# Fro116/RecommenderSystem

Measured on AMD Instinct MI355X. Metric: interactions/sec, higher is better.
Workload: dtype bf16

## Files before the change

include/rsys_debug.h:

```cpp
#ifndef RSYS_DEBUG_H
#define RSYS_DEBUG_H
#include "rsys.h"

#ifdef __cplusplus
extern "C" {
#endif

int32_t rsys_debug_get(rsys_model* m, const char* key, void* out, int64_t bytes);

int32_t rsys_local_group_create(int32_t world, int32_t device, void** group);
int32_t rsys_local_group_destroy(void* group);
int32_t rsys_comm_init_local(void* group, int32_t rank, rsys_comm** out);
int32_t rsys_comm_debug_delay(rsys_comm* c, int32_t microseconds);

int32_t rsys_dev_alloc(void** p, size_t bytes);
int32_t rsys_dev_free(void* p);
int32_t rsys_dev_h2d(void* dst, const void* src, size_t bytes);
int32_t rsys_dev_d2h(void* dst, const void* src, size_t bytes);
int32_t rsys_dev_memset(void* dst, int value, size_t bytes);
int32_t rsys_op_gemm(int32_t dtype, const void* A, const void* B, void* C, int32_t M, int32_t N, int32_t K,
                     int64_t lda, int64_t ldb, int64_t ldc, int32_t a_km, int32_t b_km, int32_t a_f32, int32_t c_f32,
                     int32_t splitk);
int32_t rsys_op_gemm_rows(int32_t dtype, const void* A, const void* B, void* C, int32_t M, int32_t N, int32_t K,
                          int64_t lda, int64_t ldb, int64_t ldc, int32_t b_km, int32_t c_f32, const int32_t* rows_dev);
int32_t rsys_op_gemm_klimit(int32_t dtype, const void* A, const void* B, void* C, int32_t M, int32_t N, int32_t K,
                            int64_t lda, int64_t ldb, int64_t ldc, int32_t accumulate, const int32_t* k_dev);
int32_t rsys_op_gemm_epi(int32_t dtype, const void* A, const void* B, void* C, int32_t M, int32_t N, int32_t K, int64_t lda,
                         int64_t ldb, int64_t ldc, int32_t b_km, int32_t c_f32, int32_t epi, float alpha, int32_t accum,
                         const float* bias, const float* resid, int64_t ldr, void* C2, int64_t ldc2, const float* E,
                         const float* rope_cos, const float* rope_sin, const float* rope_cs, const int32_t* rope_pos, int32_t T,
                         int32_t hd, int32_t n_q, int32_t n_k, const int32_t* m_dev, char* tag, int32_t tag_bytes, int32_t* half);
int32_t rsys_debug_gemm_route(int32_t dtype, int32_t M, int32_t N, int32_t K, int64_t lda, int64_t ldb, int64_t ldc, int32_t a_km,
                              int32_t b_km, int32_t a_f32, int32_t c_f32, int32_t epi, int32_t splitk, int32_t flags, float alpha,
                              int32_t accum, int32_t set, int32_t m_expect, int32_t cus, char* tag, int32_t tag_bytes, int32_t* splits);
int32_t rsys_op_attention(int32_t dtype, int32_t B, int32_t T, int32_t H, int32_t KV, int32_t hd, const void* qkv,
                          const int32_t* uid, const int32_t* tm, void* O, float* lse, const void* dO, void* dqkv,
                          const float* rope_cos, const float* rope_sin);
int32_t rsys_op_attention_ex(int32_t dtype, int32_t B, int32_t T, int32_t H, int32_t KV, int32_t hd, const void* qkv,
                             const int32_t* uid, const int32_t* tm, void* O, float* lse, const void* dO, void* dqkv,
                             const float* rope_cos, const float* rope_sin, const int32_t* rope_pos, int32_t rope_rows,
                             const int32_t* q_active, float* amax_fwd, float* amax_bwd);
int32_t rsys_op_attention_selected(int32_t dtype, int32_t B, int32_t T, int32_t H, int32_t KV, int32_t hd, const void* qkv,
                                   const int32_t* uid, const int32_t* tm, int32_t n_sel, const int32_t* sel, void* O);
int32_t rsys_op_attention_cached(int32_t dtype, int32_t rows, int32_t T, int32_t H, int32_t KV, int32_t hd, const void* qkv, const void* cache,
                                 int32_t n_slots, const int32_t* slot, const int32_t* n_hist, const int32_t* n_cand, void* O);
// ... 103 lines not shown
```

recommendersystem_amd/_lib.py:

```python
import ctypes as C
import os

os.environ.setdefault("HSA_ENABLE_IPC_MODE_LEGACY", "0")

HERE = os.path.dirname(os.path.abspath(__file__))
LIB_PATH = os.path.join(HERE, "librsys_hip.so")


class RsysError(RuntimeError):
    pass


class rsys_config(C.Structure):
    _fields_ = [
        ("num_layers", C.c_int32), ("num_heads", C.c_int32), ("num_kv_heads", C.c_int32),
        ("embed_dim", C.c_int32), ("intermediate_dim", C.c_int32), ("max_sequence_length", C.c_int32),
        ("vocab_0", C.c_int32), ("vocab_1", C.c_int32),
        ("vocab_status", C.c_int32), ("vocab_gender", C.c_int32), ("vocab_source", C.c_int32),
        ("metadata_dim", C.c_int32),
        ("min_ts", C.c_double), ("max_ts", C.c_double),
        ("rating_mean", C.c_float), ("rating_std", C.c_float), ("mask_rate", C.c_float),
        ("mask_topk", C.c_int32), ("finetune", C.c_int32), ("finetune_metric", C.c_int32),
        ("dtype", C.c_int32), ("max_rows", C.c_int32), ("lora_dropout", C.c_float),
        ("table_shard_rank", C.c_int32), ("table_shard_world", C.c_int32), ("sampled_negatives", C.c_int32),
# ... 165 lines not shown
    ("rsys_grad_sync_schedule", C.c_int32, [_P, C.POINTER(C.c_int64), C.c_int32, C.POINTER(C.c_int32)]),
    ("rsys_comm_info", C.c_int32, [_P, C.POINTER(C.c_int32)]),
    ("rsys_allreduce_f64", C.c_int32, [_P, C.POINTER(C.c_double), C.c_int32]),
    ("rsys_self_test", C.c_int32, [_P]),
    ("rsys_param_checksum", C.c_int32, [_P, C.POINTER(C.c_double * 4)]),
    ("rsys_grad_buffer", C.c_int32, [_P, C.POINTER(_P), C.POINTER(C.c_int64)]),
    ("rsys_param_buffer", C.c_int32, [_P, C.POINTER(_P), C.POINTER(C.c_int64)]),
    ("rsys_refresh_shadow", C.c_int32, [_P]),
    ("rsys_dev_alloc", C.c_int32, [C.POINTER(_P), C.c_size_t]),
    ("rsys_dev_free", C.c_int32, [_P]),
    ("rsys_dev_h2d", C.c_int32, [_P, _P, C.c_size_t]),
    ("rsys_dev_d2h", C.c_int32, [_P, _P, C.c_size_t]),
    ("rsys_dev_memset", C.c_int32, [_P, C.c_int, C.c_size_t]),
    ("rsys_op_gemm", C.c_int32, [C.c_int32, _P, _P, _P, C.c_int32, C.c_int32, C.c_int32, C.c_int64, C.c_int64, C.c_int64,
                                 C.c_int32, C.c_int32, C.c_int32, C.c_int32, C.c_int32]),
    ("rsys_op_f8_quantize", C.c_int32, [_P, C.c_int64, C.c_int32, C.c_int32, C.c_int32, C.c_int32, C.c_int32, C.c_int32, _P, C.c_int64, _P, _P, _P,
                                          C.c_int32, C.c_int32, C.c_int32]),
    ("rsys_op_f8_weights", C.c_int32, [_P, C.c_int64, C.c_int32, C.c_int32, C.c_int32, C.c_int32, C.c_int32, _P, _P, _P, C.c_int64]),
    ("rsys_op_gemm_f8", C.c_int32, [_P, _P, _P, C.c_int32, C.c_int32, C.c_int32, C.c_int64, C.c_int64, C.c_int64, C.c_int32, C.c_int32, _P,
                                      C.c_int32, C.c_int32, C.c_int32, C.c_int32, C.c_int32]),
    ("rsys_op_gemm_rows", C.c_int32, [C.c_int32, _P, _P, _P, C.c_int32, C.c_int32, C.c_int32, C.c_int64, C.c_int64, C.c_int64,
                                      C.c_int32, C.c_int32, _P]),
    ("rsys_op_gemm_klimit", C.c_int32, [C.c_int32, _P, _P, _P, C.c_int32, C.c_int32, C.c_int32, C.c_int64, C.c_int64, C.c_int64, C.c_int32, _P]),
    ("rsys_op_gemm_epi", C.c_int32, [C.c_int32, _P, _P, _P, C.c_int32, C.c_int32, C.c_int32, C.c_int64, C.c_int64, C.c_int64, C.c_int32, C.c_int32,
                                     C.c_int32, C.c_float, C.c_int32, _P, _P, C.c_int64, _P, C.c_int64, _P, _P, _P, _P, _P,
                                     C.c_int32, C.c_int32, C.c_int32, C.c_int32, _P, C.c_char_p, C.c_int32, C.POINTER(C.c_int32)]),
    ("rsys_debug_gemm_route", C.c_int32, [C.c_int32] * 4 + [C.c_int64] * 3 + [C.c_int32] * 7 + [C.c_float] + [C.c_int32] * 4
                                          + [C.c_char_p, C.c_int32, C.POINTER(C.c_int32)]),
    ("rsys_op_attention", C.c_int32, [C.c_int32] + [C.c_int32] * 5 + [_P] * 9),
    ("rsys_op_attention_ex", C.c_int32, [C.c_int32] + [C.c_int32] * 5 + [_P] * 10 + [C.c_int32, _P, _P, _P]),
    ("rsys_op_query_weights", C.c_int32, [_P, C.c_int64, _P, _P, _P, C.c_int32, _P, C.c_int32, _P, _P, C.c_int32, C.c_int32,
                                          _P, _P, _P, _P, _P, _P, C.c_float, C.c_int32, _P,
                                          _P, _P, _P, C.c_int32, _P, _P, C.c_int32, _P, _P]),
    ("rsys_op_topk", C.c_int32, [_P, C.c_int64, C.c_int32, C.c_int32, C.c_int32, _P, _P, _P]),
    ("rsys_op_topk_window", C.c_int32, [_P, C.c_int64, C.c_int32, C.c_int32, _P, _P, _P, _P, _P, _P, _P]),
    ("rsys_op_lse", C.c_int32, [_P, C.c_int64, C.c_int32, C.c_int32, _P]),
    ("rsys_op_target_rank", C.c_int32, [_P, C.c_int64, C.c_int32, C.c_int32, _P, _P]),
    ("rsys_op_pair_ranks", C.c_int32, [_P, C.c_int64, C.c_int32, C.c_int32, _P, _P, _P, _P]),
    ("rsys_rank_gram_get", C.c_int32, [_P, C.c_int32, C.c_int32, _P, _P, _P, C.c_int64]),
    ("rsys_op_rerank", C.c_int32, [C.c_int32, C.c_int32, _P, _P, _P, _P, _P, _P]),
    ("rsys_op_embedding_scatter", C.c_int32, [_P, C.c_int64, _P, _P, C.c_int32, C.c_int32, C.c_int32, _P, C.c_int32]),
    ("rsys_op_rmsnorm_fwd", C.c_int32, [C.c_int32, _P, _P, _P, _P, C.c_int64, C.c_int32, _P, _P, _P]),
    ("rsys_op_rmsnorm_bwd", C.c_int32, [C.c_int32, C.c_int32] + [_P] * 11 + [C.c_int64, C.c_int32, _P, C.c_int32]),
    ("rsys_op_ce", C.c_int32, [C.c_int32, _P, C.c_int64, C.c_int32, C.c_int32] + [_P] * 6 + [C.c_float, _P, C.c_int32]),
    ("rsys_op_rating_tail", C.c_int32, [C.c_int32, _P, _P, C.c_int32, C.c_int32] + [_P] * 6 + [C.c_float, C.c_float, C.c_int32]
                                        + [_P] * 5 + [C.c_int32]),
# ... 77 lines not shown
```

recommendersystem_amd/csrc/capi.hip:

```cpp
#include <algorithm>
#include <dlfcn.h>
#include <math.h>
#include <stdlib.h>
#include <string.h>

#include <sstream>

#include "comm.hpp"
#include "encoder_handle.hpp"
#include "model_internal.hpp"

namespace rsys {
static thread_local std::string g_err;
void set_error(const std::string& msg) { g_err = msg; }
}

using namespace rsys;

struct rsys_model { Model* m; };
struct rsys_optimizer { Optimizer o; };

#define CHECK_HANDLE(h) do { if ((h) == nullptr) { set_error("null handle"); return RSYS_ERR_ARG; } } while (0)

namespace {
// ... 829 lines not shown
  return RSYS_OK;
}
int32_t rsys_param_buffer(rsys_model* h, void** p, int64_t* n) { CHECK_HANDLE(h); *p = h->m->P; *n = h->m->n_total; return RSYS_OK; }
int32_t rsys_refresh_shadow(rsys_model* h) { CHECK_HANDLE(h); return model_refresh_shadow(h->m); }

int32_t rsys_dev_alloc(void** p, size_t bytes) { HIP_CHECK(hipMalloc(p, bytes ? bytes : 16)); HIP_CHECK(hipMemset(*p, 0, bytes ? bytes : 16)); return RSYS_OK; }
int32_t rsys_dev_free(void* p) { HIP_CHECK(hipFree(p)); return RSYS_OK; }
int32_t rsys_dev_h2d(void* d, const void* s, size_t n) { HIP_CHECK(hipMemcpy(d, s, n, hipMemcpyHostToDevice)); return RSYS_OK; }
int32_t rsys_dev_d2h(void* d, const void* s, size_t n) { HIP_CHECK(hipDeviceSynchronize()); HIP_CHECK(hipMemcpy(d, s, n, hipMemcpyDeviceToHost)); return RSYS_OK; }
int32_t rsys_dev_memset(void* d, int v, size_t n) { HIP_CHECK(hipMemset(d, v, n)); return RSYS_OK; }

int32_t rsys_op_gemm(int32_t dtype, const void* A, const void* B, void* C, int32_t M, int32_t N, int32_t K, int64_t lda,
                     int64_t ldb, int64_t ldc, int32_t a_km, int32_t b_km, int32_t a_f32, int32_t c_f32, int32_t splitk) {
  switches_parse();
  GemmParams p{};
  p.A = A; p.B = B; p.C = C; p.M = M; p.N = N; p.K = K; p.lda = lda; p.ldb = ldb; p.ldc = ldc;
  p.c_f32 = c_f32; p.splitk = splitk < 1 ? 1 : splitk; p.alpha = 1.f;
  p.epi = p.splitk > 1 ? EPI_ATOMIC : EPI_STORE;
  if (sw().debug_epi >= 0) p.epi = sw().debug_epi;
  int rc = dtype == RSYS_DTYPE_BF16 ? launch_gemm<bf16>(p, a_f32 != 0, false, a_km != 0, b_km != 0, nullptr)
                                    : launch_gemm<float>(p, false, false, a_km != 0, b_km != 0, nullptr);
  if (rc) return rc;
  HIP_CHECK(hipDeviceSynchronize());
  return RSYS_OK;
}

int32_t rsys_op_gemm_rows(int32_t dtype, const void* A, const void* B, void* C, int32_t M, int32_t N, int32_t K, int64_t lda,
                          int64_t ldb, int64_t ldc, int32_t b_km, int32_t c_f32, const int32_t* rows_dev) {
  switches_parse();
  ARG_CHECK(rows_dev != nullptr, "rsys_op_gemm_rows: rows_dev is null");
  GemmParams p{};
  p.A = A; p.B = B; p.C = C; p.M = M; p.N = N; p.K = K; p.lda = lda; p.ldb = ldb; p.ldc = ldc;
  p.c_f32 = c_f32 != 0; p.splitk = 1; p.alpha = 1.f; p.epi = EPI_STORE; p.m_dev = rows_dev;
  if (c_f32 == 3) { p.epi = EPI_ATOMIC; p.splitk = 8; }
  int rc = dtype == RSYS_DTYPE_BF16 ? launch_gemm<bf16>(p, false, false, false, b_km != 0, nullptr)
                                    : launch_gemm<float>(p, false, false, false, b_km != 0, nullptr);
  if (rc) return rc;
  HIP_CHECK(hipDeviceSynchronize());
  return RSYS_OK;
}

int32_t rsys_op_gemm_klimit(int32_t dtype, const void* A, const void* B, void* C, int32_t M, int32_t N, int32_t K, int64_t lda,
                            int64_t ldb, int64_t ldc, int32_t accumulate, const int32_t* k_dev) {
  switches_parse();
  ARG_CHECK(k_dev != nullptr, "rsys_op_gemm_klimit: k_dev is null");
  GemmParams p{};
// ... 963 lines not shown
```

recommendersystem_amd/csrc/gemm.hpp:

```cpp
#pragma once
#include "common.hpp"

namespace rsys {

enum GemmEpi : int {
  EPI_STORE = 0,
  EPI_ACCUM = 1,
  EPI_ATOMIC = 2,
  EPI_BIAS = 3,
  EPI_RESIDUAL = 4,
  EPI_QKV_ROPE = 5,
  EPI_SWIGLU = 6,
  EPI_TABLE = 7,
  EPI_GELU = 8,
  EPI_SWIGLU_BWD = 9
};

enum GemmFlag : int {
  GEMM_NO_STORE_ALLOWANCE = 1 << 0,
  GEMM_ONE_WG_PER_TILE = 1 << 1,
  GEMM_START_STAGGER = 1 << 2,
  GEMM_BAND_SHIFT = 3,
  GEMM_BAND_MASK = 15 << GEMM_BAND_SHIFT,
  GEMM_SPLITK_256 = 1 << 7,
// ... 27 lines not shown
  int f8_seg_cols;
  int f8_alt;
  int f8_kb[3];
  float* f8_amax_out;
  int f8_rseg;
  int f8_rowmode;
};

template <typename CT>
int launch_gemm(const GemmParams& p, bool a_f32, bool b_f32, bool a_km, bool b_km, hipStream_t s);

enum GemmKernel : int { GK_NT, GK_NN, GK_TN, GK_8P, GK_8C, GK_4P, GK_8T, GK_4K, GK_8TS, GK_8S, GK_8M, GK_COUNT };
extern const char* const gemm_kernel_tags[GK_COUNT];
struct GemmRoute { GemmKernel kernel; int splitk; };
template <typename CT>
GemmRoute gemm_route(const GemmParams& p, bool a_f32, bool b_f32, bool a_km, bool b_km, int cus);

template <typename CT>
long long gemm_slab_need(const GemmParams& p, bool a_f32, bool b_f32, bool a_km, bool b_km);

struct GemmGroupPlan;
bool gemm8p_group_eligible(const GemmParams& p);
int gemm8p_group_plan_create(const GemmParams* probs, int n, GemmGroupPlan** out, bool ordered = false);
void gemm8p_group_plan_destroy(GemmGroupPlan* pl);
double gemm8p_group_flops(const GemmGroupPlan* pl);
bool gemm8p_group_on_4k(const GemmGroupPlan* pl);
int gemm8p_group_splitk(const GemmGroupPlan* pl);
int launch_gemm8p_group(const GemmGroupPlan* pl, hipStream_t s);

bool gemm8p_mix_eligible(const GemmParams& p);
int launch_gemm8p_mix(const GemmParams& p, hipStream_t s);
bool gemm8p_f8_eligible(const GemmParams& p);
int launch_gemm8p_f8(const GemmParams& p, hipStream_t s);
bool gemm8p_f8_splitk_eligible(const GemmParams& p);
int launch_gemm8p_f8_splitk(const GemmParams& p, hipStream_t s);

const char* gemm_kernel_name(const GemmParams& p, bool bf16_mode, bool a_f32, bool b_f32, bool a_km, bool b_km);
bool gemm8c_uses_half(const GemmParams& p, int cus);

}
```

recommendersystem_amd/csrc/gemm8p.hip:

```cpp
#include <algorithm>
#include <vector>

#include "gemm.hpp"
#include "gemm_epi.hpp"
#include "gemm_epi_reg.hpp"

namespace rsys {

#define GLB_AS __attribute__((address_space(1)))

namespace {

constexpr int T8_BM = 256, T8_BN = 256, T8_BK = 64;

typedef __attribute__((ext_vector_type(4))) int i32x4;
extern "C" __device__ void rsys_raw_buffer_load_lds(i32x4 rsrc, LDS_AS unsigned int* lds, int size, int voffset, int soffset,
                                                    int offset, int aux) __asm("llvm.amdgcn.raw.buffer.load.lds");

__device__ __forceinline__ i32x4 make_rsrc(const char* base) {
  const unsigned long long a = (unsigned long long)base;
  i32x4 r;
  r[0] = __builtin_amdgcn_readfirstlane((int)(unsigned int)a);
  r[1] = __builtin_amdgcn_readfirstlane((int)(unsigned int)((a >> 32) & 0xFFFFu));
  r[2] = -1;
// ... 495 lines not shown
  bool asm4k = false;
  double flops = 0.0;
  float* slab_all = nullptr; size_t slab_bytes = 0; int max_mn4 = 0;
};

__global__ void slab_reduce_group_kernel(const GemmParams* __restrict__ probs) {
  const GemmParams& p = probs[blockIdx.y];
  const long long n4 = (long long)p.M * p.N / 4, stride = (long long)p.M * p.N;
  float* C = (float*)p.C;
  for (long long i = (long long)blockIdx.x * blockDim.x + threadIdx.x; i < n4; i += (long long)gridDim.x * blockDim.x) {
    float4 acc = *(const float4*)(p.slab + 4 * i);
    for (int sp = 1; sp < p.splitk; ++sp) {
      const float4 v = *(const float4*)(p.slab + sp * stride + 4 * i);
      acc.x += v.x; acc.y += v.y; acc.z += v.z; acc.w += v.w;
    }
    const long long e = 4 * i, row = e / p.N; const int col = (int)(e % p.N);
    float4* c = (float4*)(C + row * p.ldc + col);
    float4 o = *c; o.x += acc.x; o.y += acc.y; o.z += acc.z; o.w += acc.w; *c = o;
  }
}

bool gemm8p_group_eligible(const GemmParams& p) { return (p.f8 ? gemm8p_f8_splitk_eligible(p) : gemm8p_tn_eligible(p)) && p.slab == nullptr; }

int gemm8p_group_plan_create(const GemmParams* probs, int n, GemmGroupPlan** out, bool ordered) {
  ARG_CHECK(n >= 1 && n <= 128, "grouped GEMM: 1..128 products");
  const int per_xcd = std::max(1, cu_count() / 8);
  std::vector<int> tiles(n), ktiles(n);
  int ktmax = 0;
  const bool f8 = probs[0].f8 != 0;
  for (int i = 0; i < n; ++i) {
    ARG_CHECK((probs[i].f8 != 0) == f8, "grouped GEMM: fp8 and bf16 products in one plan");
    ARG_CHECK(gemm8p_group_eligible(probs[i]), "grouped GEMM: product not eligible for the split-K LDS-DMA kernel");
    tiles[i] = ((probs[i].M + T8_BM - 1) / T8_BM) * ((probs[i].N + T8_BN - 1) / T8_BN);
    ARG_CHECK(tiles[i] < 65536, "grouped GEMM: too many tiles");
    ktiles[i] = f8 ? probs[i].K / 128 : (probs[i].K + T8_BK - 1) / T8_BK;
    ktmax = std::max(ktmax, ktiles[i]);
  }
  std::vector<int> order(n);
  for (int i = 0; i < n; ++i) order[i] = i;
  std::stable_sort(order.begin(), order.end(), [&](int a, int b) { return (long long)tiles[a] * ktiles[a] > (long long)tiles[b] * ktiles[b]; });
  std::vector<std::vector<int>> lists(8);
  long long load[8] = {0, 0, 0, 0, 0, 0, 0, 0};
  for (int i : order) {
    int best = 0;
    for (int x = 1; x < 8; ++x) if (load[x] < load[best]) best = x;
    lists[best].push_back(i); load[best] += (long long)tiles[i] * ktiles[i];
  }
  const int force = sw().debug_8g_splitk;
  int best_s = 1; double best_t = 1e300;
  for (int s = 1; s <= 16; ++s) {
    if (s > 1 && (ktmax + s - 1) / s < 8) break;
    double worst = 0.0;
    for (int x = 0; x < 8; ++x) {
      std::vector<double> slot(per_xcd, 0.0);
      for (int i : lists[x]) {
        const int per = (ktiles[i] + s - 1) / s;
        for (int sp = 0; sp < s; ++sp) {
          const int nt = std::min(ktiles[i], (sp + 1) * per) - sp * per;
          if (nt <= 0) continue;
          for (int t = 0; t < tiles[i]; ++t) { auto it = std::min_element(slot.begin(), slot.end()); *it += nt + 24.0; }
        }
      }
      worst = std::max(worst, *std::max_element(slot.begin(), slot.end()));
    }
    if (worst < best_t) { best_t = worst; best_s = s; }
  }
  if (force > 0) best_s = std::min(force, 255);
  std::vector<GemmParams> hp(probs, probs + n);
  std::vector<int> off(9, 0);
  std::vector<unsigned int> work;
  int longest = 0;
  double flops = 0.0;
  for (int i = 0; i < n; ++i) { hp[i].splitk = best_s; if (hp[i].alpha == 0.f) hp[i].alpha = 1.f; flops += 2.0 * hp[i].M * hp[i].N * (double)hp[i].K; }
  float* slab_all = nullptr; size_t slab_bytes = 0; int max_mn4 = 0;
  if (ordered) {
    ARG_CHECK(!f8, "grouped GEMM: the ordered form exists for the bf16 products only");
    long long total = 0;
    for (int i = 0; i < n; ++i) {
      ARG_CHECK(hp[i].N % 4 == 0 && hp[i].ldc % 4 == 0, "grouped GEMM: the ordered split-K sum needs N % 4 == 0");
      total += (long long)best_s * hp[i].M * hp[i].N;
      max_mn4 = std::max(max_mn4, (int)((long long)hp[i].M * hp[i].N / 4));
    }
    slab_bytes = (size_t)total * 4;
    if (hipMalloc((void**)&slab_all, slab_bytes) != hipSuccess) { set_error("grouped GEMM: hipMalloc of the split-K slabs failed"); return RSYS_ERR_HIP; }
    long long at = 0;
    for (int i = 0; i < n; ++i) { hp[i].slab = slab_all + at; hp[i].slab_floats = (long long)best_s * hp[i].M * hp[i].N; at += hp[i].slab_floats; }
  }
  for (int x = 0; x < 8; ++x) {
    off[x] = (int)work.size();
    for (int i : lists[x]) {
      const int per = (ktiles[i] + best_s - 1) / best_s;
      for (int sp = 0; sp < best_s; ++sp) {
        if (sp * per >= ktiles[i]) continue;
        for (int t = 0; t < tiles[i]; ++t) work.push_back(((unsigned int)i << 24) | ((unsigned int)sp << 16) | (unsigned int)t);
      }
    }
    longest = std::max(longest, (int)work.size() - off[x]);
  }
  off[8] = (int)work.size();
  GemmGroupPlan* pl = new GemmGroupPlan();
  const size_t b_probs = (sizeof(GemmParams) * n + 255) / 256 * 256, b_off = 256, b_work = (work.size() * 4 + 255) / 256 * 256;
  pl->slab_all = slab_all; pl->slab_bytes = slab_bytes; pl->max_mn4 = max_mn4;
  if (hipMalloc(&pl->dev, b_probs + b_off + b_work) != hipSuccess) { if (slab_all) hipFree(slab_all); delete pl; set_error("grouped GEMM: hipMalloc failed"); return RSYS_ERR_HIP; }
  pl->d_probs = (const GemmParams*)pl->dev; pl->d_off = (const int*)((char*)pl->dev + b_probs); pl->d_work = (const unsigned int*)((char*)pl->dev + b_probs + b_off);
  bool ok = hipMemcpy((void*)pl->d_probs, hp.data(), sizeof(GemmParams) * n, hipMemcpyHostToDevice) == hipSuccess;
  ok = ok && hipMemcpy((void*)pl->d_off, off.data(), 9 * 4, hipMemcpyHostToDevice) == hipSuccess;
  ok = ok && hipMemcpy((void*)pl->d_work, work.data(), work.size() * 4, hipMemcpyHostToDevice) == hipSuccess;
  if (!ok) { hipFree(pl->dev); if (slab_all) hipFree(slab_all); delete pl; set_error("grouped GEMM: plan upload failed"); return RSYS_ERR_HIP; }
  pl->grid = 8 * longest; pl->n = n; pl->splitk = best_s; pl->flops = flops; pl->f8 = f8;
  pl->asm4k = !f8;
  for (int i = 0; i < n && pl->asm4k; ++i) pl->asm4k = gemm4k_eligible(hp[i]);
  *out = pl;
  return RSYS_OK;
}
void gemm8p_group_plan_destroy(GemmGroupPlan* pl) { if (pl) { if (pl->dev) hipFree(pl->dev); if (pl->slab_all) hipFree(pl->slab_all); delete pl; } }
double gemm8p_group_flops(const GemmGroupPlan* pl) { return pl->flops; }
bool gemm8p_group_on_4k(const GemmGroupPlan* pl) { return pl->asm4k && !pl->f8 && sw().gemm4k != 0; }
int gemm8p_group_splitk(const GemmGroupPlan* pl) { return pl->splitk; }
int launch_gemm8p_group(const GemmGroupPlan* pl, hipStream_t s) {
  if (pl->grid <= 0) return RSYS_OK;
  if (pl->slab_all) HIP_CHECK(hipMemsetAsync(pl->slab_all, 0, pl->slab_bytes, s));
  if (pl->f8) hipLaunchKernelGGL(gemm8p_group_f8_kernel, dim3(pl->grid), dim3(512), 0, s, pl->d_probs, pl->d_off, pl->d_work);
// ... 176 lines not shown
```

recommendersystem_amd/csrc/model.hip:

```cpp
#include "model_internal.hpp"

namespace rsys {

static void add_tensor(Model* m, const std::string& name, int64_t rows, int64_t cols, int ndim, int64_t off, int64_t ld,
                       int map, bool trainable = true, bool frozen = false) {
  TensorInfo t{name, rows, cols, ndim, off, ld, map, trainable, frozen};
  m->by_name[name] = (int)m->tensors.size();
  m->tensors.push_back(t);
}

static void build_layout(Model* m) {
  const int D = m->D, Ip = m->Ip, I = m->I, L = m->L, hd = m->hd, H = m->H, KV = m->KV;
  const bool ft = m->cfg.finetune != 0;
  int64_t off = 0;
  auto take = [&](int64_t n) { int64_t o = off; off += pad8(n); return o; };
  m->lo.resize(L);
  if (ft) {
    for (int l = 0; l < L; ++l) { m->lo[l].la = take((int64_t)16 * D); m->lo[l].lb = take((int64_t)m->Nqkv * 16); }
  }
  const int64_t n_lora = off;
  m->o_status = take((m->cfg.vocab_status + 1) * 16);
  m->o_gender = take((m->cfg.vocab_gender + 1) * 4);
  m->o_source = take((m->cfg.vocab_source + 1) * 4);
  m->o_lin_w = take((int64_t)D * 32);
// ... 94 lines not shown
  m->L = cfg->num_layers; m->H = cfg->num_heads; m->KV = cfg->num_kv_heads; m->D = cfg->embed_dim;
  m->I = cfg->intermediate_dim; m->Ip = m->fp8 ? (m->I + 127) / 128 * 128 : (m->I + 15) / 16 * 16;
  m->Sa = cfg->max_sequence_length; m->Ta = 2 * m->Sa; set_row_len(m, m->Sa);
  m->V0 = cfg->vocab_0; m->V1 = cfg->vocab_1; m->V = m->V0 + m->V1; m->M = cfg->metadata_dim;
  m->Mp = (m->M + 63) / 64 * 64; m->K = cfg->mask_topk; m->hd = hd;
  m->Nqkv = (m->H + 2 * m->KV) * hd; m->rows_max = cfg->max_rows;
  m->sharded = cfg->table_shard_world >= 1;
  m->sh_world = m->sharded ? cfg->table_shard_world : 1; m->sh_rank = m->sharded ? cfg->table_shard_rank : 0;
  if (m->sh_world > 16 || m->sh_rank < 0 || m->sh_rank >= m->sh_world || (m->sharded && cfg->finetune)) {
    delete m;
    set_error("table_shard: rank must be in [0, world), world <= 16, and finetuning keeps the table replicated (it is frozen)");
    return RSYS_ERR_ARG;
  }
  m->row_lo = (int)((int64_t)m->sh_rank * (m->V + 1) / m->sh_world);
  m->TR = (int)((int64_t)(m->sh_rank + 1) * (m->V + 1) / m->sh_world) - m->row_lo;
  HIP_CHECK(hipStreamCreateWithFlags(&m->stream, hipStreamNonBlocking));
  build_layout(m);
  const int64_t D = m->D, N = (int64_t)m->rows_max * m->Sa, NT = 2 * N, KB = (int64_t)m->K * m->rows_max;
  const size_t e = m->esz;
  DALLOC(m->P, m->n_total * 4); DALLOC(m->G, m->n_total * 4);
  if (m->bf16_mode) { DALLOC(m->Sh, m->n_total * 2); DALLOC(m->ShT, m->n_total * 2); } else { m->Sh = m->P; }
  DALLOC(m->Meta, (int64_t)m->TR * m->Mp * e);
  DALLOC(m->F32, (int64_t)m->TR * D * 4); DALLOC(m->FT, (int64_t)m->TR * D * e);
  if (m->bf16_mode) {
    m->Vp = ((int64_t)m->TR + 63) / 64 * 64;
    DALLOC(m->MetaT, (int64_t)m->Mp * m->Vp * 2); DALLOC(m->dFT, (int64_t)D * m->Vp * 2);
    HIP_CHECK(hipMemset(m->MetaT, 0, (size_t)m->Mp * m->Vp * 2)); HIP_CHECK(hipMemset(m->dFT, 0, (size_t)D * m->Vp * 2));
  }
  {
    const int half = hd / 2;
    std::vector<float> c((size_t)m->Ta * half), s((size_t)m->Ta * half);
    for (int k = 0; k < half; ++k) {
      float freq = 1.0f / powf(500000.0f, (float)(2 * k) / (float)hd);
      for (int t = 0; t < m->Ta; ++t) { float a = (float)t * freq; c[(size_t)t * half + k] = cosf(a); s[(size_t)t * half + k] = sinf(a); }
    }
    DALLOC(m->rope_cos, c.size() * 4); DALLOC(m->rope_sin, s.size() * 4); DALLOC(m->rope_cs, c.size() * 8);
    HIP_CHECK(hipMemcpy(m->rope_cos, c.data(), c.size() * 4, hipMemcpyHostToDevice));
    HIP_CHECK(hipMemcpy(m->rope_sin, s.data(), s.size() * 4, hipMemcpyHostToDevice));
    std::vector<float> cs(c.size() * 2);
    for (size_t i = 0; i < c.size(); ++i) { cs[2 * i] = c[i]; cs[2 * i + 1] = s[i]; }
    HIP_CHECK(hipMemcpy(m->rope_cs, cs.data(), cs.size() * 4, hipMemcpyHostToDevice));
    m->rope_npos = m->Ta;
  }
  {
    size_t per_i = 4 * 6 + 8 + 4 * 2 + 18 * 4  + 4 * 3 + 4 * 2 + 12 * 4 ;
    DALLOC(m->batch_blob, (size_t)N * per_i + 4096);
    unsigned char* p = (unsigned char*)m->batch_blob;
    auto carve = [&](size_t bytes) { void* r = p; p += (bytes + 15) / 16 * 16; return r; };
    BatchDev& b = m->bd;
    b.time = (const double*)carve(N * 8);
    b.userid = (const int*)carve(N * 4); b.tmid = (const int*)carve(N * 4); b.gender = (const int*)carve(N * 4);
// ... 256 lines not shown
    }
    if (t.ld != t.cols) {
      std::vector<float> host((size_t)rows * t.ld);
      HIP_CHECK(hipStreamSynchronize(m->stream));
      HIP_CHECK(hipMemcpy(host.data(), m->P + t.off, host.size() * 4, hipMemcpyDeviceToHost));
      for (int64_t r = 0; r < rows; ++r)
        for (int64_t c = t.cols; c < t.ld; ++c) host[r * t.ld + c] = 0.f;
      HIP_CHECK(hipMemcpy(m->P + t.off, host.data(), host.size() * 4, hipMemcpyHostToDevice));
    }
    if (t.map == MAP_W1 && m->Ip != m->I) {
      for (int64_t r = m->I; r < m->Ip; ++r) {
        HIP_CHECK(hipMemsetAsync(m->P + t.off + ((r / 16) * 32 + (r % 16)) * t.ld, 0, t.ld * 4, m->stream));
        HIP_CHECK(hipMemsetAsync(m->P + t.off + ((r / 16) * 32 + 16 + (r % 16)) * t.ld, 0, t.ld * 4, m->stream));
      }
    }
    if (t.name.find("embedding.weight") != std::string::npos)
      HIP_CHECK(hipMemsetAsync(m->P + t.off + (t.rows - 1) * t.ld, 0, t.cols * 4, m->stream));
  }
  RC(model_refresh_shadow(m));
  HIP_CHECK(hipStreamSynchronize(m->stream));
  return RSYS_OK;
}

static int build_meta_t(Model* m) {
  m->table_dirty = true;
  if (!m->bf16_mode) return RSYS_OK;
  TransposeBatch b; b.n = 1;
  b.job[0].src = (const bf16*)m->Meta; b.job[0].dst = (bf16*)m->MetaT; b.job[0].rows = m->TR; b.job[0].cols = m->Mp;
  b.job[0].ld_src = m->Mp; b.job[0].ld_dst = m->Vp;
  RC(launch_transpose_bf16(b, m->stream));
  HIP_CHECK(hipStreamSynchronize(m->stream));
  return RSYS_OK;
}

static int meta_write_rows(Model* m, const float* rows, int64_t nrows) {
  const int64_t Mdim = m->M;
  HIP_CHECK(hipSetDevice(m->device));
  const int64_t chunk = 4096;
  std::vector<float> hostf((size_t)chunk * m->Mp);
  std::vector<unsigned short> hosth;
  if (m->bf16_mode) hosth.resize((size_t)chunk * m->Mp);
  HIP_CHECK(hipMemset(m->Meta, 0, (size_t)m->TR * m->Mp * m->esz));
  for (int64_t r0 = 0; r0 < nrows; r0 += chunk) {
    int64_t nr = std::min(chunk, nrows - r0);
    for (int64_t r = 0; r < nr; ++r) {
      const float* src = rows + (r0 + r) * Mdim;
      if (m->bf16_mode) {
        unsigned short* d = hosth.data() + r * m->Mp;
        for (int64_t c = 0; c < Mdim; ++c) {
          uint32_t u; memcpy(&u, &src[c], 4);
          uint32_t rb = ((u >> 16) & 1u) + 0x7FFFu;
          d[c] = (unsigned short)((u + rb) >> 16);
        }
        for (int64_t c = Mdim; c < m->Mp; ++c) d[c] = 0;
      } else {
        float* d = hostf.data() + r * m->Mp;
        memcpy(d, src, Mdim * 4);
        for (int64_t c = Mdim; c < m->Mp; ++c) d[c] = 0.f;
      }
    }
    void* dst = (unsigned char*)m->Meta + (size_t)r0 * m->Mp * m->esz;
    HIP_CHECK(hipMemcpy(dst, m->bf16_mode ? (void*)hosth.data() : (void*)hostf.data(), (size_t)nr * m->Mp * m->esz, hipMemcpyHostToDevice));
  }
  return build_meta_t(m);
}

int model_load_metadata(Model* m, const float* table, int64_t V, int64_t Mdim) {
  ARG_CHECK(V == m->V && Mdim == m->M, "metadata table shape must be (V, metadata_dim)");
  const int64_t nrows = std::max<int64_t>(0, std::min<int64_t>(m->row_lo + m->TR, m->V) - m->row_lo);
  return meta_write_rows(m, table + (int64_t)m->row_lo * Mdim, nrows);
}

int model_random_metadata(Model* m, uint64_t seed) {
  HIP_CHECK(hipSetDevice(m->device));
  HIP_CHECK(hipMemsetAsync(m->Meta, 0, (size_t)m->TR * m->Mp * m->esz, m->stream));
  const float std_ = 1.0f / sqrtf((float)m->M);
  const long long nrows = std::max<long long>(0, std::min<long long>(m->row_lo + m->TR, m->V) - m->row_lo);
  if (m->bf16_mode) RC(launch_fill_normal_t<bf16>((bf16*)m->Meta, nrows, m->M, m->Mp, std_, seed, m->stream, m->row_lo));
  else RC(launch_fill_normal_t<float>((float*)m->Meta, nrows, m->M, m->Mp, std_, seed, m->stream, m->row_lo));
  HIP_CHECK(hipStreamSynchronize(m->stream));
  return build_meta_t(m);
}

int model_set_rope(Model* m, const float* c, const float* s, int64_t n_pos) {
  ARG_CHECK(n_pos == m->Ta, "rope tables must have 2*max_sequence_length positions");
  HIP_CHECK(hipSetDevice(m->device));
  size_t bytes = (size_t)n_pos * (m->hd / 2) * 4;
  HIP_CHECK(hipMemcpy(m->rope_cos, c, bytes, hipMemcpyHostToDevice));
  HIP_CHECK(hipMemcpy(m->rope_sin, s, bytes, hipMemcpyHostToDevice));
  {
    const size_t n = bytes / 4;
    std::vector<float> cs(n * 2);
    for (size_t i = 0; i < n; ++i) { cs[2 * i] = c[i]; cs[2 * i + 1] = s[i]; }
    HIP_CHECK(hipMemcpy(m->rope_cs, cs.data(), cs.size() * 4, hipMemcpyHostToDevice));
  }
  return RSYS_OK;
}

int model_param_io(Model* m, const char* name, float* out, const float* in, int64_t n, int which) {
  auto it = m->by_name.find(name);
  if (it == m->by_name.end()) { set_error(std::string("unknown parameter: ") + name); return RSYS_ERR_ARG; }
  const TensorInfo& t = m->tensors[it->second];
  ARG_CHECK(n == t.rows * t.cols, "element count does not match the parameter's shape");
  HIP_CHECK(hipSetDevice(m->device));
// ... 551 lines not shown
```

recommendersystem_amd/csrc/model.hpp:

```cpp
#pragma once
#include <functional>
#include <map>
#include <string>
#include <vector>

#include "../../include/rsys.h"
#include "../../include/rsys_debug.h"
#include "comm.hpp"
#include "gemm.hpp"
#include "kernels.hpp"
#include "workspace.hpp"

namespace rsys {

enum RowMap { MAP_DIRECT = 0, MAP_W1 = 1, MAP_W3 = 2 };

struct TensorInfo {
  std::string name;
  int64_t rows, cols;
  int ndim;
  int64_t off;
  int64_t ld;
  int map;
  bool trainable;
// ... 68 lines not shown
  unsigned char* W8 = nullptr;
  unsigned char* W8T = nullptr;
  float* f8_wamax = nullptr;
  float* f8_aamax = nullptr;
  float* f8_desc = nullptr;
  unsigned char* a8 = nullptr;
  void* f8_jobs = nullptr; int* f8_tile_job = nullptr; int* f8_tile_first = nullptr; int f8_ntiles = 0;
  bool w8_dirty = true;
  void* sel_scratch = nullptr;
  float* rope_cs = nullptr;
  bool f8_dw = false;
  bool f8_tcopies = true;
  struct F8T { unsigned char *xn, *O, *hn, *g, *gxt, *dab, *dht, *dqkv; };
  std::vector<F8T> f8t;
  float* f8_desc_dw = nullptr;
  int64_t f8_ldt = 0;
  float* f8_dw_stage = nullptr;
  int64_t f8_dw_stage_base = 0;
  std::vector<void*> f8_keep;
  bool table_dirty = true;
  void* Meta = nullptr;
  float* F32 = nullptr;
  void* FT = nullptr;
  void* MetaT = nullptr; void* dFT = nullptr; int64_t Vp = 0;
  bool sharded = false; int sh_rank = 0, sh_world = 1;
  int row_lo = 0, TR = 0;
  rsys_comm* shard_comm = nullptr;
  int *u_slot = nullptr, *u_ids = nullptr, *u_tok = nullptr, *u_plan = nullptr , *u_bound = nullptr, *u_off = nullptr;
  int U = 0, uV = 0;
  std::vector<long long> need_off, serve_off, need_offD, serve_offD;
  int* req_ids = nullptr; long long req_cap = 0, R = 0;
  float *Frem = nullptr; float* rows_xchg = nullptr; long long xchg_cap = 0;
  void *EwAll = nullptr, *EwC = nullptr; float *metaOwn = nullptr, *metaAll = nullptr, *metaC = nullptr, *vp_max = nullptr, *vp_lmax = nullptr, *vp_sums = nullptr;
  int *vp_nlive = nullptr, *vp_pre = nullptr; float* dEwC = nullptr;
  float* metaAllT[2] = {nullptr, nullptr};
  int* h_counts = nullptr;
  hipEvent_t ev_counts = nullptr; bool counts_pending = false;
  int host_stream_syncs = 0, host_event_waits = 0;
  int64_t ldl_loc = 0; float* sumsq_E = nullptr;
  int* ss_cols = nullptr; void* ss_F = nullptr; float *ss_dF = nullptr, *ss_tl = nullptr, *ss_dt = nullptr;
  unsigned int* ss_bitmap = nullptr; int* ss_tcount = nullptr;
  unsigned long long cur_seed = 0, cur_step = 0;
  float *rope_cos = nullptr, *rope_sin = nullptr;
  int rope_npos = 0;
  std::vector<void*> allocs;
  BatchDev bd;
  void* batch_blob = nullptr;
// ... 263 lines not shown
```

recommendersystem_amd/csrc/model_backward.hip:

```cpp
#include "model_internal.hpp"

namespace rsys {

static int ensure_transposes(Model* m) {
  if (!m->bf16_mode || !m->wt_dirty) return RSYS_OK;
  const int D = m->D, Ip = m->Ip;
  TransposeBatch b; b.n = 0;
  auto add = [&](int64_t off, int rows, int cols, long long ld) -> int {
    TransposeJob& j = b.job[b.n++];
    j.src = (const bf16*)m->Sh + off; j.dst = (bf16*)m->ShT + off; j.rows = rows; j.cols = cols; j.ld_src = ld; j.ld_dst = rows;
    if (b.n == 64) { int rc = launch_transpose_bf16(b, m->stream); b.n = 0; return rc; }
    return RSYS_OK;
  };
  for (int l = 0; l < m->L; ++l) {
    RC(add(m->lo[l].wqkv, m->Nqkv, D, D));
    RC(add(m->lo[l].wo, D, D, D));
    RC(add(m->lo[l].w13, 2 * Ip, D, D));
    RC(add(m->lo[l].w2, D, Ip, Ip));
  }
  RC(launch_transpose_bf16(b, m->stream));
  m->wt_dirty = false;
  return RSYS_OK;
}

// ... 339 lines not shown
  {
    GemmParams p{};
    p.A = gxt + D; p.lda = 2 * D; p.B = m->feat; p.ldb = 32; p.C = m->G + m->o_lin_w; p.ldc = 32; p.c_f32 = 1;
    p.M = D; p.N = 32; p.K = N; p.epi = EPI_ATOMIC;
    RC(gemm<T>(m, "gemm_action_dw", p, false, true, true));
  }
  RC(launch_colsum_add(gx + D, 2 * D, N, D, m->G + m->o_lin_b, s));
  {
    GemmParams p{};
    p.A = gxt + D; p.lda = 2 * D; p.B = W<T>(m, m->o_lin_w); p.ldb = 32; p.C = m->gf; p.ldc = 32; p.c_f32 = 1;
    p.M = N; p.N = 32; p.K = D; p.epi = EPI_STORE;
    RC(gemm<T>(m, "gemm_action_dx", p, false, false, true));
  }
  SmallParams sp = small_params(m);
  RC(launch_action_small_bwd(m->gf, b, sp, m->G + m->o_pcos, m->G + m->o_psin, m->G + m->o_status, m->G + m->o_gender,
                             m->G + m->o_source, s));
  toc(m);
  return RSYS_OK;
}

template <typename T>
static int finalize_grads_t(Model* m, int stage) {
  tic(m, stage == 2 ? "phase_table_bwd_gemm" : "phase_table_bwd");
  const bool direct = m->bf16_mode && m->D % 64 == 0;
  if (stage != 2 && direct) {
    RC(launch_cast_transpose_colsum(m->G + m->o_E, (bf16*)m->dFT, m->TR, m->D, m->Vp, m->G + m->o_bp, m->stream));
  } else if (stage != 2) {
    m->table_dirty = true;
    const bool fused = m->bf16_mode && m->D <= 1024 && 1024 % (m->D >> 2) == 0;
    if (fused) {
      RC(launch_cast_colsum(m->G + m->o_E, (bf16*)m->FT, m->TR, m->D, m->G + m->o_bp, m->stream));
    } else {
      if (m->bf16_mode) RC(launch_cast<bf16>(m->G + m->o_E, (bf16*)m->FT, (long long)m->TR * m->D, m->stream));
      RC(launch_colsum_add(m->G + m->o_E, m->D, m->TR, m->D, m->G + m->o_bp, m->stream));
    }
    if (m->bf16_mode) {
      TransposeBatch b; b.n = 1;
      b.job[0].src = (const bf16*)m->FT; b.job[0].dst = (bf16*)m->dFT; b.job[0].rows = m->TR; b.job[0].cols = m->D;
      b.job[0].ld_src = m->D; b.job[0].ld_dst = m->Vp;
      RC(launch_transpose_bf16(b, m->stream));
    }
  }
  if (stage != 1) {
    GemmParams p{};
    p.C = m->G + m->o_Wp; p.ldc = m->Mp; p.c_f32 = 1; p.M = m->D; p.N = m->Mp; p.epi = EPI_ATOMIC;
    if (m->bf16_mode) {
      p.A = m->dFT; p.lda = m->Vp; p.B = m->MetaT; p.ldb = m->Vp; p.K = (int)m->Vp;
      RC(gemm<T>(m, "gemm_table_dw", p, false, false, false));
    } else {
      p.A = m->G + m->o_E; p.lda = m->D; p.B = m->Meta; p.ldb = m->Mp; p.K = m->TR;
      RC(gemm<T>(m, "gemm_table_dw", p, false, true, true));
    }
  }
  toc(m);
  return RSYS_OK;
}

int model_finalize_grads(Model* m) {
  if (!m->table_grads_pending || m->cfg.finetune) return RSYS_OK;
  DetScope det(m);
  m->table_grads_pending = false;
  return m->bf16_mode ? finalize_grads_t<bf16>(m, 0) : finalize_grads_t<float>(m, 0);
}

bool model_finalize_splittable(const Model* m) { return m->table_grads_pending && !m->cfg.finetune && m->bf16_mode; }

int model_split_table_enable(Model* m, int on) {
  if (!on) { m->split_table = false; m->table_head_hook = nullptr; return RSYS_OK; }
  ARG_CHECK(!m->sharded, "split table reduce: the item table is row-sharded (its rows are reduced by their owners already)");
  ARG_CHECK(m->bf16_mode && !m->cfg.finetune, "split table reduce: bf16 training of the full model only (the fp32 mode's metadata-projection gradient reads G[E] itself)");
  HIP_CHECK(hipSetDevice(m->device));
  if (!m->tbl_R) {
    const int64_t N = (int64_t)m->rows_max * m->Sa;
    m->tok_cap = N + 1;
    DALLOC(m->tbl_R, (int64_t)m->TR * m->D * 4);
// ... 73 lines not shown
```

Before: 1.651 million.

## Drop transposed table-gradient buffers and run the table dW GEMM on row-major operands

The bf16 table-gradient path no longer keeps transposed, padded copies of the metadata (MetaT) and the gradient (dFT), and no longer uses the fused cast-transpose-colsum kernel. It casts the fp32 gradient into a row-major bf16 buffer and runs the dW GEMM with K-major operands over TR rows. This removes the transpose kernel and the metadata transpose after loads, at the cost of relying on the K-major GEMM path, which may be less efficient for this shape. It also factors the grouped-GEMM work dealing into a separate function and adds debug and test entry points.

```diff
diff --git a/include/rsys_debug.h b/include/rsys_debug.h
--- a/include/rsys_debug.h
+++ b/include/rsys_debug.h
@@ -21,6 +21,10 @@
 int32_t rsys_op_gemm(int32_t dtype, const void* A, const void* B, void* C, int32_t M, int32_t N, int32_t K,
                      int64_t lda, int64_t ldb, int64_t ldc, int32_t a_km, int32_t b_km, int32_t a_f32, int32_t c_f32,
                      int32_t splitk);
+int32_t rsys_op_gemm_group(int32_t n, const void* const* A, const void* const* B, void* const* C, const int32_t* M, const int32_t* N,
+                           const int32_t* K, const int64_t* lda, const int64_t* ldb, const int64_t* ldc, int32_t ordered);
+int32_t rsys_debug_group_deal(int32_t n, const int32_t* M, const int32_t* N, const int32_t* K, int32_t cus, int32_t* splits_out,
+                              int32_t* off_out, int32_t* work_out, int64_t cap, int64_t* n_work_out);
 int32_t rsys_op_gemm_rows(int32_t dtype, const void* A, const void* B, void* C, int32_t M, int32_t N, int32_t K,
                           int64_t lda, int64_t ldb, int64_t ldc, int32_t b_km, int32_t c_f32, const int32_t* rows_dev);
 int32_t rsys_op_gemm_klimit(int32_t dtype, const void* A, const void* B, void* C, int32_t M, int32_t N, int32_t K,
diff --git a/recommendersystem_amd/_lib.py b/recommendersystem_amd/_lib.py
--- a/recommendersystem_amd/_lib.py
+++ b/recommendersystem_amd/_lib.py
@@ -211,6 +211,8 @@
     ("rsys_op_gemm_rows", C.c_int32, [C.c_int32, _P, _P, _P, C.c_int32, C.c_int32, C.c_int32, C.c_int64, C.c_int64, C.c_int64,
                                       C.c_int32, C.c_int32, _P]),
     ("rsys_op_gemm_klimit", C.c_int32, [C.c_int32, _P, _P, _P, C.c_int32, C.c_int32, C.c_int32, C.c_int64, C.c_int64, C.c_int64, C.c_int32, _P]),
+    ("rsys_op_gemm_group", C.c_int32, [C.c_int32, _P, _P, _P, _P, _P, _P, _P, _P, _P, C.c_int32]),
+    ("rsys_debug_group_deal", C.c_int32, [C.c_int32, _P, _P, _P, C.c_int32, _P, _P, _P, C.c_int64, _P]),
     ("rsys_op_gemm_epi", C.c_int32, [C.c_int32, _P, _P, _P, C.c_int32, C.c_int32, C.c_int32, C.c_int64, C.c_int64, C.c_int64, C.c_int32, C.c_int32,
                                      C.c_int32, C.c_float, C.c_int32, _P, _P, C.c_int64, _P, C.c_int64, _P, _P, _P, _P, _P,
                                      C.c_int32, C.c_int32, C.c_int32, C.c_int32, _P, C.c_char_p, C.c_int32, C.POINTER(C.c_int32)]),
diff --git a/recommendersystem_amd/csrc/capi.hip b/recommendersystem_amd/csrc/capi.hip
--- a/recommendersystem_amd/csrc/capi.hip
+++ b/recommendersystem_amd/csrc/capi.hip
@@ -875,6 +875,48 @@
                                     : launch_gemm<float>(p, false, false, a_km != 0, b_km != 0, nullptr);
   if (rc) return rc;
   HIP_CHECK(hipDeviceSynchronize());
+  return RSYS_OK;
+}
+
+int32_t rsys_op_gemm_group(int32_t n, const void* const* A, const void* const* B, void* const* C, const int32_t* M, const int32_t* N,
+                           const int32_t* K, const int64_t* lda, const int64_t* ldb, const int64_t* ldc, int32_t ordered) {
+  switches_parse();
+  ARG_CHECK(n >= 1 && n <= 128 && A && B && C && M && N && K && lda && ldb && ldc, "rsys_op_gemm_group: 1..128 products, no null array");
+  std::vector<GemmParams> ps((size_t)n);
+  for (int i = 0; i < n; ++i) {
+    GemmParams p{};
+    p.A = A[i]; p.B = B[i]; p.C = C[i]; p.M = M[i]; p.N = N[i]; p.K = K[i]; p.lda = lda[i]; p.ldb = ldb[i]; p.ldc = ldc[i];
+    p.c_f32 = 1; p.epi = EPI_ATOMIC; p.alpha = 1.f;
+    ARG_CHECK(p.A && p.B && p.C && p.K > 0, "rsys_op_gemm_group: null operand or empty product");
+    ps[i] = p;
+  }
+  GemmGroupPlan* pl = nullptr;
+  RC(gemm8p_group_plan_create(ps.data(), n, &pl, ordered != 0));
+  int rc = launch_gemm8p_group(pl, nullptr);
+  hipError_t e = hipDeviceSynchronize();
+  gemm8p_group_plan_destroy(pl);
+  if (rc) return rc;
+  HIP_CHECK(e);
+  return RSYS_OK;
+}
+
+int32_t rsys_debug_group_deal(int32_t n, const int32_t* M, const int32_t* N, const int32_t* K, int32_t cus, int32_t* splits_out, int32_t* off_out,
+                              int32_t* work_out, int64_t cap, int64_t* n_work_out) {
+  switches_parse();
+  ARG_CHECK(n >= 1 && n <= 128 && M && N && K && splits_out && off_out && work_out && n_work_out && cus >= 8, "rsys_debug_group_deal: 1..128 products, no null array, cus >= 8");
+  std::vector<int> tiles((size_t)n), ktiles((size_t)n);
+  for (int i = 0; i < n; ++i) {
+    ARG_CHECK(M[i] > 0 && N[i] > 0 && K[i] > 0, "rsys_debug_group_deal: empty product");
+    tiles[i] = ((M[i] + 255) / 256) * ((N[i] + 255) / 256); ktiles[i] = (K[i] + 63) / 64;
+    ARG_CHECK(tiles[i] < 65536, "rsys_debug_group_deal: too many tiles");
+  }
+  std::vector<unsigned int> work; int off[9];
+  const int splits = gemm8p_group_deal(tiles.data(), ktiles.data(), n, cus, sw().debug_8g_splitk, off, work);
+  *n_work_out = (int64_t)work.size();
+  ARG_CHECK((int64_t)work.size() <= cap, "rsys_debug_group_deal: work_out too small");
+  for (int i = 0; i < n; ++i) splits_out[i] = splits;
+  for (int x = 0; x < 9; ++x) off_out[x] = off[x];
+  memcpy(work_out, work.data(), work.size() * 4);
   return RSYS_OK;
 }
 
diff --git a/recommendersystem_amd/csrc/gemm.hpp b/recommendersystem_amd/csrc/gemm.hpp
--- a/recommendersystem_amd/csrc/gemm.hpp
+++ b/recommendersystem_amd/csrc/gemm.hpp
@@ -1,4 +1,6 @@
 #pragma once
+#include <vector>
+
 #include "common.hpp"
 
 namespace rsys {
@@ -73,6 +75,7 @@
 struct GemmGroupPlan;
 bool gemm8p_group_eligible(const GemmParams& p);
 int gemm8p_group_plan_create(const GemmParams* probs, int n, GemmGroupPlan** out, bool ordered = false);
+int gemm8p_group_deal(const int* tiles, const int* ktiles, int n, int cus, int force, int off[9], std::vector<unsigned int>& work);
 void gemm8p_group_plan_destroy(GemmGroupPlan* pl);
 double gemm8p_group_flops(const GemmGroupPlan* pl);
 bool gemm8p_group_on_4k(const GemmGroupPlan* pl);
diff --git a/recommendersystem_amd/csrc/gemm8p.hip b/recommendersystem_amd/csrc/gemm8p.hip
--- a/recommendersystem_amd/csrc/gemm8p.hip
+++ b/recommendersystem_amd/csrc/gemm8p.hip
@@ -541,20 +541,10 @@
 
 bool gemm8p_group_eligible(const GemmParams& p) { return (p.f8 ? gemm8p_f8_splitk_eligible(p) : gemm8p_tn_eligible(p)) && p.slab == nullptr; }
 
-int gemm8p_group_plan_create(const GemmParams* probs, int n, GemmGroupPlan** out, bool ordered) {
-  ARG_CHECK(n >= 1 && n <= 128, "grouped GEMM: 1..128 products");
-  const int per_xcd = std::max(1, cu_count() / 8);
-  std::vector<int> tiles(n), ktiles(n);
+int gemm8p_group_deal(const int* tiles, const int* ktiles, int n, int cus, int force, int off[9], std::vector<unsigned int>& work) {
+  const int per_xcd = std::max(1, cus / 8);
   int ktmax = 0;
-  const bool f8 = probs[0].f8 != 0;
-  for (int i = 0; i < n; ++i) {
-    ARG_CHECK((probs[i].f8 != 0) == f8, "grouped GEMM: fp8 and bf16 products in one plan");
-    ARG_CHECK(gemm8p_group_eligible(probs[i]), "grouped GEMM: product not eligible for the split-K LDS-DMA kernel");
-    tiles[i] = ((probs[i].M + T8_BM - 1) / T8_BM) * ((probs[i].N + T8_BN - 1) / T8_BN);
-    ARG_CHECK(tiles[i] < 65536, "grouped GEMM: too many tiles");
-    ktiles[i] = f8 ? probs[i].K / 128 : (probs[i].K + T8_BK - 1) / T8_BK;
-    ktmax = std::max(ktmax, ktiles[i]);
-  }
+  for (int i = 0; i < n; ++i) ktmax = std::max(ktmax, ktiles[i]);
   std::vector<int> order(n);
   for (int i = 0; i < n; ++i) order[i] = i;
   std::stable_sort(order.begin(), order.end(), [&](int a, int b) { return (long long)tiles[a] * ktiles[a] > (long long)tiles[b] * ktiles[b]; });
@@ -565,7 +555,6 @@
     for (int x = 1; x < 8; ++x) if (load[x] < load[best]) best = x;
     lists[best].push_back(i); load[best] += (long long)tiles[i] * ktiles[i];
   }
-  const int force = sw().debug_8g_splitk;
   int best_s = 1; double best_t = 1e300;
   for (int s = 1; s <= 16; ++s) {
     if (s > 1 && (ktmax + s - 1) / s < 8) break;
@@ -585,11 +574,39 @@
     if (worst < best_t) { best_t = worst; best_s = s; }
   }
   if (force > 0) best_s = std::min(force, 255);
+  work.clear();
+  for (int x = 0; x < 8; ++x) {
+    off[x] = (int)work.size();
+    for (int i : lists[x]) {
+      const int per = (ktiles[i] + best_s - 1) / best_s;
+      for (int sp = 0; sp < best_s; ++sp) {
+        if (sp * per >= ktiles[i]) continue;
+        for (int t = 0; t < tiles[i]; ++t) work.push_back(((unsigned int)i << 24) | ((unsigned int)sp << 16) | (unsigned int)t);
+      }
+    }
+  }
+  off[8] = (int)work.size();
+  return best_s;
+}
+
+int gemm8p_group_plan_create(const GemmParams* probs, int n, GemmGroupPlan** out, bool ordered) {
+  ARG_CHECK(n >= 1 && n <= 128, "grouped GEMM: 1..128 products");
+  std::vector<int> tiles(n), ktiles(n);
+  const bool f8 = probs[0].f8 != 0;
+  for (int i = 0; i < n; ++i) {
+    ARG_CHECK((probs[i].f8 != 0) == f8, "grouped GEMM: fp8 and bf16 products in one plan");
+    ARG_CHECK(gemm8p_group_eligible(probs[i]), "grouped GEMM: product not eligible for the split-K LDS-DMA kernel");
+    tiles[i] = ((probs[i].M + T8_BM - 1) / T8_BM) * ((probs[i].N + T8_BN - 1) / T8_BN);
+    ARG_CHECK(tiles[i] < 65536, "grouped GEMM: too many tiles");
+    ktiles[i] = f8 ? probs[i].K / 128 : (probs[i].K + T8_BK - 1) / T8_BK;
+  }
+  std::vector<unsigned int> work; int off9[9];
+  const int best_s = gemm8p_group_deal(tiles.data(), ktiles.data(), n, cu_count(), sw().debug_8g_splitk, off9, work);
+  std::vector<int> off(off9, off9 + 9);
+  int longest = 0;
+  for (int x = 0; x < 8; ++x) longest = std::max(longest, off[x + 1] - off[x]);
+  double flops = 0.0;
   std::vector<GemmParams> hp(probs, probs + n);
-  std::vector<int> off(9, 0);
-  std::vector<unsigned int> work;
-  int longest = 0;
-  double flops = 0.0;
   for (int i = 0; i < n; ++i) { hp[i].splitk = best_s; if (hp[i].alpha == 0.f) hp[i].alpha = 1.f; flops += 2.0 * hp[i].M * hp[i].N * (double)hp[i].K; }
   float* slab_all = nullptr; size_t slab_bytes = 0; int max_mn4 = 0;
   if (ordered) {
@@ -605,18 +622,6 @@
     long long at = 0;
     for (int i = 0; i < n; ++i) { hp[i].slab = slab_all + at; hp[i].slab_floats = (long long)best_s * hp[i].M * hp[i].N; at += hp[i].slab_floats; }
   }
-  for (int x = 0; x < 8; ++x) {
-    off[x] = (int)work.size();
-    for (int i : lists[x]) {
-      const int per = (ktiles[i] + best_s - 1) / best_s;
-      for (int sp = 0; sp < best_s; ++sp) {
-        if (sp * per >= ktiles[i]) continue;
-        for (int t = 0; t < tiles[i]; ++t) work.push_back(((unsigned int)i << 24) | ((unsigned int)sp << 16) | (unsigned int)t);
-      }
-    }
-    longest = std::max(longest, (int)work.size() - off[x]);
-  }
-  off[8] = (int)work.size();
   GemmGroupPlan* pl = new GemmGroupPlan();
   const size_t b_probs = (sizeof(GemmParams) * n + 255) / 256 * 256, b_off = 256, b_work = (work.size() * 4 + 255) / 256 * 256;
   pl->slab_all = slab_all; pl->slab_bytes = slab_bytes; pl->max_mn4 = max_mn4;
diff --git a/recommendersystem_amd/csrc/model.hip b/recommendersystem_amd/csrc/model.hip
--- a/recommendersystem_amd/csrc/model.hip
+++ b/recommendersystem_amd/csrc/model.hip
@@ -140,11 +140,7 @@
   if (m->bf16_mode) { DALLOC(m->Sh, m->n_total * 2); DALLOC(m->ShT, m->n_total * 2); } else { m->Sh = m->P; }
   DALLOC(m->Meta, (int64_t)m->TR * m->Mp * e);
   DALLOC(m->F32, (int64_t)m->TR * D * 4); DALLOC(m->FT, (int64_t)m->TR * D * e);
-  if (m->bf16_mode) {
-    m->Vp = ((int64_t)m->TR + 63) / 64 * 64;
-    DALLOC(m->MetaT, (int64_t)m->Mp * m->Vp * 2); DALLOC(m->dFT, (int64_t)D * m->Vp * 2);
-    HIP_CHECK(hipMemset(m->MetaT, 0, (size_t)m->Mp * m->Vp * 2)); HIP_CHECK(hipMemset(m->dFT, 0, (size_t)D * m->Vp * 2));
-  }
+  if (m->bf16_mode) DALLOC(m->dF16, (int64_t)m->TR * D * 2);
   {
     const int half = hd / 2;
     std::vector<float> c((size_t)m->Ta * half), s((size_t)m->Ta * half);
@@ -447,14 +443,8 @@
   return RSYS_OK;
 }
 
-static int build_meta_t(Model* m) {
+static int meta_rows_changed(Model* m) {
   m->table_dirty = true;
-  if (!m->bf16_mode) return RSYS_OK;
-  TransposeBatch b; b.n = 1;
-  b.job[0].src = (const bf16*)m->Meta; b.job[0].dst = (bf16*)m->MetaT; b.job[0].rows = m->TR; b.job[0].cols = m->Mp;
-  b.job[0].ld_src = m->Mp; b.job[0].ld_dst = m->Vp;
-  RC(launch_transpose_bf16(b, m->stream));
-  HIP_CHECK(hipStreamSynchronize(m->stream));
   return RSYS_OK;
 }
 
@@ -487,7 +477,7 @@
     void* dst = (unsigned char*)m->Meta + (size_t)r0 * m->Mp * m->esz;
     HIP_CHECK(hipMemcpy(dst, m->bf16_mode ? (void*)hosth.data() : (void*)hostf.data(), (size_t)nr * m->Mp * m->esz, hipMemcpyHostToDevice));
   }
-  return build_meta_t(m);
+  return meta_rows_changed(m);
 }
 
 int model_load_metadata(Model* m, const float* table, int64_t V, int64_t Mdim) {
@@ -504,7 +494,7 @@
   if (m->bf16_mode) RC(launch_fill_normal_t<bf16>((bf16*)m->Meta, nrows, m->M, m->Mp, std_, seed, m->stream, m->row_lo));
   else RC(launch_fill_normal_t<float>((float*)m->Meta, nrows, m->M, m->Mp, std_, seed, m->stream, m->row_lo));
   HIP_CHECK(hipStreamSynchronize(m->stream));
-  return build_meta_t(m);
+  return meta_rows_changed(m);
 }
 
 int model_set_rope(Model* m, const float* c, const float* s, int64_t n_pos) {
diff --git a/recommendersystem_amd/csrc/model.hpp b/recommendersystem_amd/csrc/model.hpp
--- a/recommendersystem_amd/csrc/model.hpp
+++ b/recommendersystem_amd/csrc/model.hpp
@@ -114,7 +114,7 @@
   void* Meta = nullptr;
   float* F32 = nullptr;
   void* FT = nullptr;
-  void* MetaT = nullptr; void* dFT = nullptr; int64_t Vp = 0;
+  void* dF16 = nullptr;
   bool sharded = false; int sh_rank = 0, sh_world = 1;
   int row_lo = 0, TR = 0;
   rsys_comm* shard_comm = nullptr;
diff --git a/recommendersystem_amd/csrc/model_backward.hip b/recommendersystem_amd/csrc/model_backward.hip
--- a/recommendersystem_amd/csrc/model_backward.hip
+++ b/recommendersystem_amd/csrc/model_backward.hip
@@ -385,35 +385,20 @@
 template <typename T>
 static int finalize_grads_t(Model* m, int stage) {
   tic(m, stage == 2 ? "phase_table_bwd_gemm" : "phase_table_bwd");
-  const bool direct = m->bf16_mode && m->D % 64 == 0;
-  if (stage != 2 && direct) {
-    RC(launch_cast_transpose_colsum(m->G + m->o_E, (bf16*)m->dFT, m->TR, m->D, m->Vp, m->G + m->o_bp, m->stream));
-  } else if (stage != 2) {
-    m->table_dirty = true;
-    const bool fused = m->bf16_mode && m->D <= 1024 && 1024 % (m->D >> 2) == 0;
+  if (stage != 2) {
+    const bool fused = m->bf16_mode && m->D % 4 == 0 && m->D <= 1024 && 1024 % (m->D >> 2) == 0;
     if (fused) {
-      RC(launch_cast_colsum(m->G + m->o_E, (bf16*)m->FT, m->TR, m->D, m->G + m->o_bp, m->stream));
+      RC(launch_cast_colsum(m->G + m->o_E, (bf16*)m->dF16, m->TR, m->D, m->G + m->o_bp, m->stream));
     } else {
-      if (m->bf16_mode) RC(launch_cast<bf16>(m->G + m->o_E, (bf16*)m->FT, (long long)m->TR * m->D, m->stream));
+      if (m->bf16_mode) RC(launch_cast<bf16>(m->G + m->o_E, (bf16*)m->dF16, (long long)m->TR * m->D, m->stream));
       RC(launch_colsum_add(m->G + m->o_E, m->D, m->TR, m->D, m->G + m->o_bp, m->stream));
     }
-    if (m->bf16_mode) {
-      TransposeBatch b; b.n = 1;
-      b.job[0].src = (const bf16*)m->FT; b.job[0].dst = (bf16*)m->dFT; b.job[0].rows = m->TR; b.job[0].cols = m->D;
-      b.job[0].ld_src = m->D; b.job[0].ld_dst = m->Vp;
-      RC(launch_transpose_bf16(b, m->stream));
-    }
   }
   if (stage != 1) {
     GemmParams p{};
     p.C = m->G + m->o_Wp; p.ldc = m->Mp; p.c_f32 = 1; p.M = m->D; p.N = m->Mp; p.epi = EPI_ATOMIC;
-    if (m->bf16_mode) {
-      p.A = m->dFT; p.lda = m->Vp; p.B = m->MetaT; p.ldb = m->Vp; p.K = (int)m->Vp;
-      RC(gemm<T>(m, "gemm_table_dw", p, false, false, false));
-    } else {
-      p.A = m->G + m->o_E; p.lda = m->D; p.B = m->Meta; p.ldb = m->Mp; p.K = m->TR;
-      RC(gemm<T>(m, "gemm_table_dw", p, false, true, true));
-    }
+    p.A = m->bf16_mode ? (const void*)m->dF16 : (const void*)(m->G + m->o_E); p.lda = m->D; p.B = m->Meta; p.ldb = m->Mp; p.K = m->TR;
+    RC(gemm<T>(m, "gemm_table_dw", p, false, true, true));
   }
   toc(m);
   return RSYS_OK;
```

Result: no change. 1.662 million (median of 6 runs) (+0.6%).
